# mnesbit/ImageExperiments

Hardware: AMD Instinct MI355X
Metric: encode Mpixels/s at quality=3.5 (higher is better)
Workload: dtype f64; 1 GPU; 4928x3264 synthetic RGB, 8 distinct frames in turn (mt19937 seed 12345+f), quality 3.5, K=32 atoms/tile-channel, 8x8 tiles; container_bytes=6650795

## Files before the change

### imageexperiments_amd/csrc/mp_pursuit.hip

```cpp
#include <hip/hip_runtime.h>
#include <stdint.h>
#include <type_traits>

#include "mp_device.h"

namespace mpc {

namespace {

constexpr int N = 64;
constexpr int kGroups = 1;
constexpr int kWavesDouble = 12;
constexpr int kWavesFloat = 12;
constexpr int kWavesMax = 16;
constexpr int kTilesLds = kBaseFilterTiles + kBlockFilterTiles;
constexpr double W_R = 0.299, W_G = 0.587, W_B = 0.114;
constexpr double U_SCALE = 0.436 / (1.0 - 0.114);
constexpr double V_SCALE = 0.615 / (1.0 - 0.299);
#ifndef MPC_SLACK
#define MPC_SLACK 0x1p-13f
#endif
constexpr float kSlack = MPC_SLACK;
constexpr float kAbs = 0x1p-100f;
constexpr float kHuge = 1.0e30f;
#ifndef MPC_REFILL_AT
#define MPC_REFILL_AT 16
#endif
constexpr int kRefillAt = MPC_REFILL_AT;

typedef float f32x4 __attribute__((ext_vector_type(4)));
typedef short bf16x8 __attribute__((ext_vector_type(8)));

template <int COUNT, class F>
__device__ __forceinline__ void static_for(F&& f)
{
    if constexpr (COUNT > 0) {
        static_for<COUNT - 1>(f);
        f(std::integral_constant<int, COUNT - 1>{});
    }
}

__device__ __forceinline__ unsigned short bf16_of(float x)
{
    const __bf16 b = static_cast<__bf16>(x);
    return __builtin_bit_cast(unsigned short, b);
}

template <class Op>
__device__ __forceinline__ unsigned reduce4_u(unsigned x, Op op)
{
    const auto a = __builtin_amdgcn_permlane16_swap(x, x, false, false);
    const unsigned m = op(a[0], a[1]);
    const auto b = __builtin_amdgcn_permlane32_swap(m, m, false, false);
    return op(b[0], b[1]);
}
__device__ __forceinline__ float reduce4_max(float x)
{
    return __uint_as_float(reduce4_u(__float_as_uint(x), [](unsigned p, unsigned q) {
        return __float_as_uint(__builtin_amdgcn_fmed3f(__uint_as_float(p), __uint_as_float(q), __builtin_inff()));
    }));
}
__device__ __forceinline__ unsigned reduce4_add(unsigned x) { return reduce4_u(x, [](unsigned p, unsigned q) { return p + q; }); }
__device__ __forceinline__ double reduce4_add(double x)
{
    unsigned lo = (unsigned)__double2loint(x), hi = (unsigned)__double2hiint(x);
    const auto a = __builtin_amdgcn_permlane16_swap(lo, lo, false, false);
    const auto b = __builtin_amdgcn_permlane16_swap(hi, hi, false, false);
    const double m = __hiloint2double((int)b[0], (int)a[0]) + __hiloint2double((int)b[1], (int)a[1]);
    lo = (unsigned)__double2loint(m); hi = (unsigned)__double2hiint(m);
    const auto c = __builtin_amdgcn_permlane32_swap(lo, lo, false, false);
    const auto d = __builtin_amdgcn_permlane32_swap(hi, hi, false, false);
    return __hiloint2double((int)d[0], (int)c[0]) + __hiloint2double((int)d[1], (int)c[1]);
}
__device__ __forceinline__ double from_prev16(double x)
{
    const unsigned lo = (unsigned)__double2loint(x), hi = (unsigned)__double2hiint(x);
    const auto a = __builtin_amdgcn_permlane16_swap(lo, lo, false, false);
    const auto b = __builtin_amdgcn_permlane16_swap(hi, hi, false, false);
    return __hiloint2double((int)b[0], (int)a[0]);
}
__device__ __forceinline__ double from_next16(double x)
{
    const unsigned lo = (unsigned)__double2loint(x), hi = (unsigned)__double2hiint(x);
    const auto a = __builtin_amdgcn_permlane16_swap(lo, lo, false, false);
    const auto b = __builtin_amdgcn_permlane16_swap(hi, hi, false, false);
    return __hiloint2double((int)b[1], (int)a[1]);
}
__device__ __forceinline__ double from_prev32(double x)
{
    const unsigned lo = (unsigned)__double2loint(x), hi = (unsigned)__double2hiint(x);
    const auto a = __builtin_amdgcn_permlane32_swap(lo, lo, false, false);
    const auto b = __builtin_amdgcn_permlane32_swap(hi, hi, false, false);
    return __hiloint2double((int)b[0], (int)a[0]);
}
__device__ __forceinline__ double from_next32(double x)
{
    const unsigned lo = (unsigned)__double2loint(x), hi = (unsigned)__double2hiint(x);
    const auto a = __builtin_amdgcn_permlane32_swap(lo, lo, false, false);
    const auto b = __builtin_amdgcn_permlane32_swap(hi, hi, false, false);
    return __hiloint2double((int)b[1], (int)a[1]);
}

__device__ __forceinline__ float from_prev16(float x) { return __uint_as_float(__builtin_amdgcn_permlane16_swap(__float_as_uint(x), __float_as_uint(x), false, false)[0]); }
__device__ __forceinline__ float from_next16(float x) { return __uint_as_float(__builtin_amdgcn_permlane16_swap(__float_as_uint(x), __float_as_uint(x), false, false)[1]); }
__device__ __forceinline__ float from_prev32(float x) { return __uint_as_float(__builtin_amdgcn_permlane32_swap(__float_as_uint(x), __float_as_uint(x), false, false)[0]); }
__device__ __forceinline__ float from_next32(float x) { return __uint_as_float(__builtin_amdgcn_permlane32_swap(__float_as_uint(x), __float_as_uint(x), false, false)[1]); }

__device__ __forceinline__ int pos_of(int h) { return h ^ (h >> 1); }

template <class T>
__device__ __forceinline__ T chain_sum(const T (&term)[16], int h)
{
    T t = 0;
#pragma unroll
    for (int i = 0; i < 16; ++i) t += term[i];
    T u = from_prev16(t);
#pragma unroll
    for (int i = 0; i < 16; ++i) u += term[i];
    t = h == 1 ? u : t;
    u = from_prev32(t);
#pragma unroll
    for (int i = 0; i < 16; ++i) u += term[i];
    t = h == 3 ? u : t;
    u = from_next16(t);
#pragma unroll
    for (int i = 0; i < 16; ++i) u += term[i];
    t = h == 2 ? u : t;
    u = from_prev16(t);
    t = h == 3 ? u : t;
    u = from_next32(t);
    return h < 2 ? u : t;
}

struct TopKeys {
    float k1 = 0.0f, k2 = 0.0f;
    __device__ __forceinline__ void see(unsigned value_bits, unsigned keep_mask, unsigned code)
    {
        const unsigned key = (value_bits & keep_mask) | code;
        k2 = __builtin_amdgcn_fmed3f(k1, k2, __uint_as_float(key));
        const unsigned k1b = __float_as_uint(k1);
        k1 = __uint_as_float(k1b > key ? k1b : key);
    }
};
__device__ __forceinline__ unsigned in_vgpr(unsigned x)
{
    unsigned v;
    asm volatile("v_mov_b32 %0, %1" : "=v"(v) : "s"(x));
    return v;
}
__device__ __forceinline__ unsigned in_sgpr(unsigned x)
{
    unsigned v;
    asm volatile("s_mov_b32 %0, %1" : "=s"(v) : "s"(x));
    return v;
}
constexpr unsigned kKeepRow = 0x7FFFFF80u;
constexpr unsigned kKeepPair = 0x7FFFFE00u;

struct Survivors {
    int q0 = 0, q1 = 0, q2 = 0, q3 = 0, count = 0;
    bool overflow = false;
    __device__ __forceinline__ void push(int code)
    {
        if (count == 0) q0 = code; else if (count == 1) q1 = code; else if (count == 2) q2 = code; else if (count == 3) q3 = code;
        else overflow = true;
        if (count < 4) ++count;
    }
    __device__ __forceinline__ int at(int i) const { return i == 0 ? q0 : (i == 1 ? q1 : (i == 2 ? q2 : q3)); }
};

struct TileChannel {
    int prev_id = 0;
    int next_off = 0;
    int off0 = 0;
    int npairs = 0;
    int fresh = -1;
    unsigned pk0 = 0, pk1 = 0;
    unsigned swept = 0;
    bool has0 = false, live = false;
    double coeff = 0.0;
    int sel_g = 0;
    int step = 0;
    int t = 0;
    __device__ __forceinline__ unsigned packed(int p) const { return ((p < 2 ? pk0 : pk1) >> (16 * (p & 1))) & 0xFFFFu; }
};

__device__ __forceinline__ void load16(double (&x)[16], const double* p)
{
    const double2* q = reinterpret_cast<const double2*>(p);
#pragma unroll
    for (int i = 0; i < 8; ++i) {
        const double2 v = q[i];
        x[2 * i] = v.x;
        x[2 * i + 1] = v.y;
// ... 18 lines not shown

template <class T>
__device__ __forceinline__ void keep_better(T& v, int& i, int& sel, T ov, int oi, int osel)
{
    const T a = abs_of(ov), b = abs_of(v);
    if (oi >= 0 && (a > b || (a == b && i >= 0 && oi < i))) {
        v = ov; i = oi; sel = osel;
    }
}

__device__ __forceinline__ int lane_id_fresh()
{
    int l;
    asm volatile("v_mbcnt_lo_u32_b32 %0, -1, 0\n\tv_mbcnt_hi_u32_b32 %0, -1, %0" : "=v"(l));
    return l;
}
#define FRESH_LANE                                                                    \
    const int lane = lane_id_fresh();                                                 \
    const int slot = lane & 15, h = lane >> 4;                                        \
    const int pix0 = 16 * pos_of(h);                                                  \
    (void)slot; (void)h; (void)pix0;

#ifdef MPC_STAMPS
#define STAMP(i)                                              \
    {                                                         \
        __builtin_amdgcn_sched_barrier(0);                    \
        const unsigned long long now_ = __builtin_amdgcn_s_memtime(); \
        __builtin_amdgcn_sched_barrier(0);                    \
        stamp_acc[i] += now_ - stamp_prev;                    \
        stamp_prev = now_;                                    \
    }
#define COUNT(i, n) stamp_acc[i] += (unsigned long long)(n);
#else
#define STAMP(i)
#define COUNT(i, n)
#endif

}

template <class T, int kWaves>
__global__ __launch_bounds__(64 * kWaves, kWaves / 4) void mp_pursuit_kernel(const PursuitArgs a)
{
    constexpr bool kFast = std::is_same<T, float>::value;
#ifdef MPC_STAMPS
    unsigned long long stamp_acc[24];
    for (int i = 0; i < 24; ++i) stamp_acc[i] = 0;
    unsigned long long stamp_prev = __builtin_amdgcn_s_memtime();
    const unsigned long long wg_begin = __builtin_amdgcn_s_memrealtime();
#endif
    __shared__ uint4 s_tiles[kTilesLds * 256];
    __shared__ int s_rows[512], s_rowoff[512];
    __shared__ unsigned s_touch[64 * kWaves];
    __shared__ double s_quant[3][kMaxDeviceK];
    __shared__ int s_home;
    __shared__ int s_on[3];
    const int ch_first = a.n_tc[0] > 0 ? 0 : (a.n_tc[1] > 0 ? 1 : 2);
    const T* const base_rows = reinterpret_cast<const T*>(kFast ? static_cast<const void*>(a.base32) : static_cast<const void*>(a.base));
    {
        const uint16_t* const blk0 = ch_first == 0 ? a.block_tiles[0] : (ch_first == 1 ? a.block_tiles[1] : a.block_tiles[2]);
        const uint4* src_base = reinterpret_cast<const uint4*>(a.base_tiles);
        const uint4* src_blk0 = reinterpret_cast<const uint4*>(blk0);
        for (int i = threadIdx.x; i < kTilesLds * 256; i += 64 * kWaves)
            s_tiles[i] = i < kBaseFilterTiles * 256 ? src_base[i] : src_blk0[i - kBaseFilterTiles * 256];
        for (int i = threadIdx.x; i < 512; i += 64 * kWaves) {
            s_rows[i] = i < a.num_base ? a.block_rows[i] : 0;
            s_rowoff[i] = i < a.num_base ? a.block_row_off[i] : 0;
        }
        for (int i = threadIdx.x; i < 3 * kMaxDeviceK; i += 64 * kWaves)
            s_quant[i / kMaxDeviceK][i % kMaxDeviceK] = (i % kMaxDeviceK) < a.K ? a.quant[(i / kMaxDeviceK) * a.K + i % kMaxDeviceK] : 1.0;
        if (threadIdx.x == 0) {
            s_home = ch_first;
            s_on[0] = s_on[1] = s_on[2] = 0;
            s_on[ch_first] = kWaves;
        }
    }
    __syncthreads();

    const int wave = __builtin_amdgcn_readfirstlane((int)(threadIdx.x >> 6));
    int ch = ch_first;
    const T* detail = nullptr;
    const uint16_t* block_tiles = nullptr;
    const float* gram = nullptr;
    unsigned* queue = nullptr;
    long long n_tc = 0;
    auto bind_channel = [&](int c) {
        c = __builtin_amdgcn_readfirstlane(c);
        ch = c;
        detail = reinterpret_cast<const T*>(kFast ? static_cast<const void*>(c == 0 ? a.detail32[0] : (c == 1 ? a.detail32[1] : a.detail32[2]))
                                                  : static_cast<const void*>(c == 0 ? a.detail[0] : (c == 1 ? a.detail[1] : a.detail[2])));
        block_tiles = c == 0 ? a.block_tiles[0] : (c == 1 ? a.block_tiles[1] : a.block_tiles[2]);
        gram = c == 0 ? a.gram[0] : (c == 1 ? a.gram[1] : a.gram[2]);
        queue = a.queue + c;
        n_tc = c == 0 ? a.n_tc[0] : (c == 1 ? a.n_tc[1] : a.n_tc[2]);
    };
    bind_channel(ch_first);
    const long long wave_global = (long long)blockIdx.x * kWaves + wave;
    float* const my_p = a.pair_p + wave_global * (kGroups * 16 * kMaxPairs * 64);
    unsigned* const my_meta = a.pair_meta + wave_global * (kGroups * 16 * kMaxPairs * 2);
    float* const my_e = a.pair_e + wave_global * (kGroups * 16 * kMaxPairs);
    unsigned* const my_touch = s_touch + 64 * wave;
    const int K = a.K;

    const unsigned keep_row_mask = in_vgpr(kKeepRow), keep_pair_mask = in_vgpr(kKeepPair);
    unsigned n_mfma = 0, n_steps = 0;
    int unit[kGroups];
    T r[kGroups][16];
    TileChannel tc[kGroups];
#pragma unroll
    for (int g = 0; g < kGroups; ++g) {
        unit[g] = -1;
#pragma unroll
        for (int i = 0; i < 16; ++i) r[g][i] = 0;
    }
    bool queue_empty = false;

    auto tile_mfma = [&](const uint4 (&av)[4], const bf16x8 (&hi)[2], const bf16x8 (&lo)[2]) {
        f32x4 acc = {0.0f, 0.0f, 0.0f, 0.0f};
#pragma unroll
        for (int kk = 0; kk < 2; ++kk) {
            bf16x8 ah, al;
            __builtin_memcpy(&ah, &av[2 * kk + 0], 16);
            __builtin_memcpy(&al, &av[2 * kk + 1], 16);
            acc = __builtin_amdgcn_mfma_f32_16x16x32_bf16(ah, hi[kk], acc, 0, 0, 0);
            acc = __builtin_amdgcn_mfma_f32_16x16x32_bf16(ah, lo[kk], acc, 0, 0, 0);
            acc = __builtin_amdgcn_mfma_f32_16x16x32_bf16(al, hi[kk], acc, 0, 0, 0);
        }
        return acc;
    };
    auto rec_of = [&](int t) { return a.vec_in ? (long long)t : (long long)t * 3 + ch; };
    auto lds_tile = [&](uint4 (&dst)[4], int t, int lane) {
#pragma unroll
        for (int q = 0; q < 4; ++q) dst[q] = s_tiles[t * 256 + q * 64 + lane];
    };
    auto far_tile = [&](uint4 (&dst)[4], int t, int lane) {
        const uint4* tiles = reinterpret_cast<const uint4*>(block_tiles) + lane;
#pragma unroll
        for (int q = 0; q < 4; ++q) dst[q] = tiles[t * 256 + q * 64];
    };

    TopKeys tp[kGroups];
    float lbmax[kGroups];
    bool oddp[kGroups];
    float rbound[kGroups];
#pragma unroll
    for (int g = 0; g < kGroups; ++g) { lbmax[g] = -3.0e38f; oddp[g] = false; rbound[g] = 0.0f; }
    auto pair_update = [&](auto gc, auto same_p, int p, bool upd, unsigned info, float4 (&pv)[4], const float4 (&gv)[4], float E) {
        constexpr int g = decltype(gc)::value;
        FRESH_LANE
        const long long pi = (long long)(g * 16 + slot) * kMaxPairs + p;
        const int rows = (int)((info >> 9) & 127u);
        if (upd) {
            const float c32 = (float)tc[g].coeff;
            float4* pp = reinterpret_cast<float4*>(my_p + pi * 64 + 4 * h);
#pragma unroll
            for (int t = 0; t < 4; ++t) {
                pv[t].x = fmaf(-c32, gv[t].x, pv[t].x);
                pv[t].y = fmaf(-c32, gv[t].y, pv[t].y);
                pv[t].z = fmaf(-c32, gv[t].z, pv[t].z);
                pv[t].w = fmaf(-c32, gv[t].w, pv[t].w);
                pp[4 * t] = pv[t];
            }
            E = (E + 0x1p-21f * (fabsf(c32) + rbound[g])) * 1.000001f;
            if (h == 0) my_e[pi] = E;
            oddp[g] = oddp[g] || !(fabsf(c32) < kHuge);
        }
        oddp[g] = oddp[g] || !(E < kHuge);
        const bool pad2 = h == 3 && rows < 63, pad3 = h == 3 && rows < 64;
        const unsigned keepp = keep_pair_mask;
        float biggest = 0.0f;
#pragma unroll
        for (int t = 0; t < 4; ++t) {
            const float vals[4] = {pv[t].x, pv[t].y, pv[t].z, pv[t].w};
#pragma unroll
            for (int v = 0; v < 4; ++v) {
                const float m = fabsf(vals[v]);
                float ub = m + E;
                if (t == 3 && v == 2) ub = pad2 ? 0.0f : ub;
                if (t == 3 && v == 3) ub = pad3 ? 0.0f : ub;
                const unsigned code = (unsigned)((p << 4) | (t << 2) | v);
                tp[g].see(__float_as_uint(ub), keepp, decltype(same_p)::value ? in_sgpr((unsigned)__builtin_amdgcn_readfirstlane((int)code)) : code);
                biggest = __builtin_amdgcn_fmed3f(biggest, m, __builtin_inff());
            }
        }
        lbmax[g] = __builtin_amdgcn_fmed3f(lbmax[g], biggest - E, __builtin_inff());
    };
    for (;;) {
        bool any_unit = false;
        for (;;) {
        static_for<kGroups>([&](auto gc) {
            constexpr int g = decltype(gc)::value;
            if (queue_empty) return;
            const unsigned free_slots = (unsigned)(__ballot(!tc[g].live) & 0xFFFFull);
            const int n_free = __popc(free_slots);
            if (!(n_free >= kRefillAt || (unit[g] < 0 && n_free > 0))) return;
            FRESH_LANE
            int first = 0;
            if (lane == 0) first = (int)atomicAdd(queue, (unsigned)n_free);
            first = __builtin_amdgcn_readfirstlane(first);
            if ((long long)first + n_free >= n_tc) queue_empty = true;
            const long long t = (long long)first + __popc(free_slots & ((1u << slot) - 1u));
            const bool take = !tc[g].live && t < n_tc;
            if (!__ballot(take)) return;
            unit[g] = 0;
            TileChannel s;
            s.live = true;
            s.t = (int)t;
            s.next_off = a.num_base;
            const long long ts = take ? t : 0;
            T fresh_r[16];
            if (a.vec_in) {
                double in[16];
                load16(in, a.vec_in + ts * N + pix0);
#pragma unroll
                for (int i = 0; i < 16; ++i) fresh_r[i] = (T)in[i];
            } else {
                const int tiles_per_frame = a.tiles_x * a.tile_rows;
                const int frame = (int)(ts / tiles_per_frame);
                const int tile = (int)(ts - (long long)frame * tiles_per_frame);
                const int tx = tile / a.tile_rows, ty = a.tile_row_begin + (tile - tx * a.tile_rows);
                if (a.out_tile_rows > 0) s.t = (frame * a.tiles_x + tx) * a.out_tile_rows + ty;
                const uint8_t* img = a.rgb + (long long)frame * a.frame_stride;
                unsigned char px[16][3];
                const bool whole = tx * 8 + 8 <= a.width && ty * 8 + 8 <= a.height;
                if (a.rgb_aligned8 && !__ballot(!whole)) {
#pragma unroll
                    for (int rr = 0; rr < 2; ++rr) {
                        const uint2* p = reinterpret_cast<const uint2*>(img + (long long)(ty * 8 + (pix0 >> 3) + rr) * a.row_stride + 24 * tx);
                        const uint2 v0 = p[0], v1 = p[1], v2 = p[2];
                        const unsigned w[6] = {v0.x, v0.y, v1.x, v1.y, v2.x, v2.y};
#pragma unroll
                        for (int b = 0; b < 24; ++b) px[8 * rr + b / 3][b % 3] = (unsigned char)((w[b >> 2] >> (8 * (b & 3))) & 0xFFu);
                    }
                } else {
// ... 73 lines not shown
            ss = reduce4_add(ss);
            nz[g] = reduce4_add(nzl ? 1u : 0u) != 0u;
            rnorm[g] = (float)__builtin_sqrt(ss) * 1.0000002f;
            Eb[g] = kSlack * rnorm[g] + kAbs;
            rbound[g] = rnorm[g];
            odd[g] = !(rnorm[g] < kHuge);
        });
        STAMP(1)

        static_for<kGroups>([&](auto gc) {
            constexpr int g = decltype(gc)::value;
            if (unit[g] < 0) return;
            const bool mine = tc[g].live && tc[g].fresh >= 0;
            unsigned long long pend = __ballot(mine) & 0xFFFFull;
            if (!pend) return;
            FRESH_LANE
            COUNT(19, __popcll(pend))
            unsigned fresh_info = 0;
            if (mine)
                fresh_info = (tc[g].fresh < 4 ? tc[g].packed(tc[g].fresh) : my_meta[2 * ((long long)(g * 16 + slot) * kMaxPairs + tc[g].fresh)]) & 0xFFFFu;
            float4 pnew[4];
#pragma unroll
            for (int t = 0; t < 4; ++t) pnew[t] = make_float4(0.0f, 0.0f, 0.0f, 0.0f);
            while (pend) {
                const int src = __builtin_ctzll(pend);
                pend &= pend - 1;
                const int blk = __builtin_amdgcn_readlane((int)(fresh_info & 511u), src);
                n_mfma += 6 * kBlockFilterTiles;
                const uint4* tiles = reinterpret_cast<const uint4*>(block_tiles) + (long long)blk * (kBlockFilterTiles * 256) + lane;
#ifndef MPC_NEWPAIR_TILES
#define MPC_NEWPAIR_TILES 2
#endif
                constexpr int kInFlight = MPC_NEWPAIR_TILES;
#pragma unroll
                for (int t2 = 0; t2 < kBlockFilterTiles; t2 += kInFlight) {
                    uint4 av[kInFlight][4];
#pragma unroll
                    for (int t = 0; t < kInFlight; ++t)
#pragma unroll
                        for (int q = 0; q < 4; ++q) av[t][q] = tiles[(t2 + t) * 256 + q * 64];
#pragma unroll
                    for (int t = 0; t < kInFlight; ++t) {
                        const f32x4 acc = tile_mfma(av[t], bh[g], bl[g]);
                        if (slot == src) pnew[t2 + t] = make_float4(acc[0], acc[1], acc[2], acc[3]);
                    }
                }
            }
            if (mine) {
                float4* dst = reinterpret_cast<float4*>(my_p + ((long long)(g * 16 + slot) * kMaxPairs + tc[g].fresh) * 64 + 4 * h);
#pragma unroll
                for (int t = 0; t < 4; ++t) dst[4 * t] = pnew[t];
                if (h == 0) my_e[(g * 16 + slot) * kMaxPairs + tc[g].fresh] = Eb[g];
                const float4 none[4] = {};
                pair_update(gc, std::false_type{}, tc[g].fresh, false, fresh_info, pnew, none, Eb[g]);
            }
        });
        STAMP(3)

        TopKeys tb[kGroups], td[kGroups];
        bool any0 = false;
#pragma unroll
        for (int g = 0; g < kGroups; ++g) any0 = any0 || (unit[g] >= 0 && __ballot(tc[g].live && tc[g].has0) != 0);
        n_mfma += 6 * kGroups * (kBaseFilterTiles + (any0 ? kBlockFilterTiles : 0));
        {
            FRESH_LANE
            uint4 ta[4];
            f32x4 acc[kGroups], prev[kGroups];
            const unsigned keep = keep_row_mask;
            auto track = [&](TopKeys (&trk)[kGroups], const f32x4 (&val)[kGroups], unsigned code0) {
                unsigned code[4];
#pragma unroll
                for (int v = 0; v < 4; ++v) code[v] = (unsigned)__builtin_amdgcn_readfirstlane((int)(code0 + v));
#pragma unroll
                for (int g = 0; g < kGroups; ++g)
#pragma unroll
                    for (int v = 0; v < 4; ++v) trk[g].see(__float_as_uint(val[g][v]), keep, code[v]);
            };
            lds_tile(ta, 0, lane);
#pragma unroll
            for (int g = 0; g < kGroups; ++g) prev[g] = tile_mfma(ta, bh[g], bl[g]);
#pragma unroll 1
            for (int t = 1; t < kBaseFilterTiles - 1; t += 2) {
                lds_tile(ta, t, lane);
#pragma unroll
                for (int g = 0; g < kGroups; ++g) acc[g] = tile_mfma(ta, bh[g], bl[g]);
                track(tb, prev, 4 * (t - 1));
                lds_tile(ta, t + 1, lane);
#pragma unroll
                for (int g = 0; g < kGroups; ++g) prev[g] = tile_mfma(ta, bh[g], bl[g]);
                track(tb, acc, 4 * t);
            }
            lds_tile(ta, kBaseFilterTiles - 1, lane);
#pragma unroll
            for (int g = 0; g < kGroups; ++g) acc[g] = tile_mfma(ta, bh[g], bl[g]);
            track(tb, prev, 4 * (kBaseFilterTiles - 2));
            track(tb, acc, 4 * (kBaseFilterTiles - 1));
            if (any0) {
#pragma unroll 1
                for (int t = 0; t < kBlockFilterTiles; ++t) {
                    if (home) lds_tile(ta, kBaseFilterTiles + t, lane);
                    else far_tile(ta, t, lane);
#pragma unroll
                    for (int g = 0; g < kGroups; ++g) acc[g] = tile_mfma(ta, bh[g], bl[g]);
                    track(td, acc, 4 * t);
                }
            }
        }
        STAMP(4)

        Survivors sv[kGroups];
        float thr_b[kGroups], Tmin[kGroups];
        bool pass2[kGroups], rescan[kGroups];
        static_for<kGroups>([&](auto gc) {
            constexpr int g = decltype(gc)::value;
            pass2[g] = false; rescan[g] = false; thr_b[g] = 0.0f; Tmin[g] = 0.0f;
            if (unit[g] < 0) return;
            FRESH_LANE
            const bool has0 = tc[g].has0, hasp = tc[g].npairs > 0;
            const float top_b = __uint_as_float(__float_as_uint(reduce4_max(tb[g].k1)) & kKeepRow);
            const float top_d = __uint_as_float(__float_as_uint(reduce4_max(td[g].k1)) & kKeepRow);
            const float lbm = reduce4_max(lbmax[g]);
            const bool bad = odd[g] || (hasp && reduce4_add(oddp[g] ? 1u : 0u) != 0u);
            float t = top_b - Eb[g];
            if (has0) t = fmaxf(t, top_d - Eb[g]);
            if (hasp) t = fmaxf(t, lbm);
            Tmin[g] = bad ? -__builtin_inff() : t;
            thr_b[g] = (Tmin[g] - Eb[g]) * (1.0f - 0x1p-15f);
            const float thr_p = Tmin[g] * (1.0f - 0x1p-13f);
            const bool live = tc[g].live && nz[g];
            const bool vague = bad || !(thr_b[g] > 0.0f);
            const bool unclear_b = vague || !(tb[g].k2 < thr_b[g]) || (has0 && !(td[g].k2 < thr_b[g]));
            const bool unclear_p = hasp && (vague || !(tp[g].k2 < thr_p));
            pass2[g] = __ballot(live && unclear_b) != 0;
            rescan[g] = live && reduce4_add(unclear_p ? 1u : 0u) != 0u;
            if (live && !pass2[g]) {
                if (!(tb[g].k1 < thr_b[g])) {
                    const unsigned code = __float_as_uint(tb[g].k1) & 127u;
                    sv[g].push((int)(16 * (code >> 2) + 4 * h + (code & 3u)));
                }
                if (has0 && !(td[g].k1 < thr_b[g])) {
                    const unsigned code = __float_as_uint(td[g].k1) & 127u;
                    sv[g].push((1 << 16) | (int)(16 * (code >> 2) + 4 * h + (code & 3u)));
                }
            }
            if (live && hasp && !rescan[g] && !(tp[g].k1 < thr_p)) {
                const unsigned code = __float_as_uint(tp[g].k1) & 511u;
                sv[g].push((2 << 16) | (int)((code >> 4) << 11) | (int)(16 * ((code >> 2) & 3u) + 4 * h + (code & 3u)));
            }
        });
        STAMP(5)

        bool any2 = false;
#pragma unroll
        for (int g = 0; g < kGroups; ++g) any2 = any2 || pass2[g];
        if (any2) {
            static_for<kGroups>([&](auto gc) { COUNT(13, pass2[decltype(gc)::value] ? 1 : 0) });
            FRESH_LANE
            uint4 cur[4], nxt[4];
            lds_tile(cur, 0, lane);
            const int last = any0 ? kTilesLds : kBaseFilterTiles;
            auto any_tile = [&](uint4 (&dst)[4], int t) {
                if (t < kBaseFilterTiles || home) lds_tile(dst, t, lane);
                else far_tile(dst, t - kBaseFilterTiles, lane);
            };
            static_for<kGroups>([&](auto gc) { n_mfma += pass2[decltype(gc)::value] ? 6 * last : 0; });
#pragma unroll 1
            for (int t = 0; t < last; ++t) {
                any_tile(nxt, t + 1 < last ? t + 1 : t);
                const bool is_base = t < kBaseFilterTiles;
                const int row0 = (is_base ? t : t - kBaseFilterTiles) * 16 + 4 * h;
                const int limit = is_base ? a.num_base : a.rows0;
                static_for<kGroups>([&](auto gc) {
                    constexpr int g = decltype(gc)::value;
                    if (!pass2[g]) return;
                    const f32x4 acc = tile_mfma(cur, bh[g], bl[g]);
                    const bool wanted = tc[g].live && nz[g] && (is_base || tc[g].has0);
#pragma unroll
                    for (int v = 0; v < 4; ++v)
                        if (wanted && !(fabsf(acc[v]) < thr_b[g]) && row0 + v < limit) sv[g].push((is_base ? 0 : (1 << 16)) | (row0 + v));
                });
#pragma unroll
                for (int q = 0; q < 4; ++q) cur[q] = nxt[q];
            }
        }
        STAMP(6)
        static_for<kGroups>([&](auto gc) {
            constexpr int g = decltype(gc)::value;
            if (unit[g] < 0 || !__ballot(rescan[g])) return;
            FRESH_LANE
            for (int p = 0; __ballot(rescan[g] && p < tc[g].npairs) != 0; ++p) {
                if (!(rescan[g] && p < tc[g].npairs)) continue;
                const long long pi = (long long)(g * 16 + slot) * kMaxPairs + p;
                const int rows = (int)((my_meta[2 * pi] >> 9) & 127u);
                const float E = my_e[pi];
                const float4* pp = reinterpret_cast<const float4*>(my_p + pi * 64 + 4 * h);
#pragma unroll
                for (int t = 0; t < 4; ++t) {
                    const float4 x = pp[4 * t];
                    const float vals[4] = {x.x, x.y, x.z, x.w};
#pragma unroll
                    for (int v = 0; v < 4; ++v) {
                        const int row = 16 * t + 4 * h + v;
                        if (row < rows && !(fabsf(vals[v]) + E < Tmin[g])) sv[g].push((2 << 16) | (p << 11) | row);
                    }
                }
            }
        });
        STAMP(7)

        T best_val[kGroups];
        int best_idx[kGroups], best_sel[kGroups];
        int c0[kGroups], c1[kGroups], c2[kGroups], total[kGroups];
        bool exhaustive[kGroups];
        const int lane7 = lane_id_fresh();
        const int slot7 = lane7 & 15, h7 = lane7 >> 4, pix7 = 16 * pos_of(h7);
#pragma unroll
        for (int g = 0; g < kGroups; ++g) {
            best_val[g] = 0; best_idx[g] = -1; best_sel[g] = 0;
            c0[g] = __shfl(sv[g].count, slot7);
            c1[g] = __shfl(sv[g].count, slot7 + 16);
            c2[g] = __shfl(sv[g].count, slot7 + 32);
            total[g] = c0[g] + c1[g] + c2[g] + __shfl(sv[g].count, slot7 + 48);
            exhaustive[g] = reduce4_add(sv[g].overflow ? 1u : 0u) != 0u;
        }
        auto resolve = [&](auto gc, int code, const T*& ptr, int& idx, int& sel) {
            constexpr int g = decltype(gc)::value;
            const int seg = code >> 16, row = code & 2047;
            if (seg == 0) { ptr = base_rows + (long long)row * N; idx = row; sel = row; }
            else if (seg == 1) { ptr = detail + (long long)row * N; idx = tc[g].off0 + row; sel = a.num_base + row; }
            else {
                const int p = (code >> 11) & 31;
                const long long pi = (long long)(g * 16 + slot7) * kMaxPairs + p;
                const unsigned meta = my_meta[2 * pi];
                const int drow = s_rowoff[meta & 511u] + row;
                ptr = detail + (long long)drow * N;
                idx = (int)(meta >> 16) + row;
                sel = a.num_base + drow;
            }
        };
        auto evaluate2 = [&](const bool (&on)[kGroups], const int (&code)[kGroups]) {
            const T* ptr[kGroups];
            int idx[kGroups], sel[kGroups];
            T x[kGroups][16];
            static_for<kGroups>([&](auto gc) {
                constexpr int g = decltype(gc)::value;
                ptr[g] = base_rows; idx[g] = -1; sel[g] = 0;
                if (on[g]) resolve(gc, code[g], ptr[g], idx[g], sel[g]);
            });
#pragma unroll
            for (int g = 0; g < kGroups; ++g) load16(x[g], ptr[g] + pix7);
#pragma unroll
            for (int g = 0; g < kGroups; ++g)
#pragma unroll
                for (int i = 0; i < 16; ++i) x[g][i] = x[g][i] * r[g][i];
            T p[kGroups];
#pragma unroll
            for (int g = 0; g < kGroups; ++g) p[g] = chain_sum(x[g], h7);
#pragma unroll
            for (int g = 0; g < kGroups; ++g)
                if (on[g]) keep_better(best_val[g], best_idx[g], best_sel[g], p[g], idx[g], sel[g]);
        };
        for (int k = 0;; ++k) {
            bool on[kGroups];
            int code[kGroups];
            bool any = false;
#pragma unroll
            for (int g = 0; g < kGroups; ++g) {
                on[g] = unit[g] >= 0 && tc[g].live && !exhaustive[g] && k < total[g];
                any = any || on[g];
                const int owner = k < c0[g] ? 0 : (k < c0[g] + c1[g] ? 1 : (k < c0[g] + c1[g] + c2[g] ? 2 : 3));
                const int local = k - (owner == 0 ? 0 : (owner == 1 ? c0[g] : (owner == 2 ? c0[g] + c1[g] : c0[g] + c1[g] + c2[g])));
                code[g] = __shfl(sv[g].at(local & 3), slot7 + 16 * owner);
            }
            if (!__ballot(any)) break;
            COUNT(14, 1)
            evaluate2(on, code);
        }
// ... 14 lines not shown
                    bool on[kGroups];
                    int code[kGroups];
                    bool more = false, any = false;
                    static_for<kGroups>([&](auto gc) {
                        constexpr int g = decltype(gc)::value;
                        on[g] = ex[g] && n < n_all[g];
                        more = more || on[g];
                        code[g] = 0;
                        if (n < a.num_base) code[g] = n;
                        else if (n < a.num_base + 64) { code[g] = (1 << 16) | (n - a.num_base); on[g] = on[g] && tc[g].has0 && n - a.num_base < a.rows0; }
                        else {
                            const int p = (n - a.num_base - 64) >> 6, row = (n - a.num_base - 64) & 63;
                            code[g] = (2 << 16) | (p << 11) | row;
                            if (on[g]) on[g] = row < (int)((my_meta[2 * ((long long)(g * 16 + slot7) * kMaxPairs + p)] >> 9) & 127u);
                        }
                        any = any || on[g];
                    });
                    if (!__ballot(more)) break;
                    if (!__ballot(any)) continue;
                    evaluate2(on, code);
                }
            }
        }
        STAMP(9)

        T xrow[kGroups][16];
#pragma unroll
        for (int g = 0; g < kGroups; ++g) {
            FRESH_LANE
            const int sg = (unit[g] >= 0 && tc[g].live && best_idx[g] >= 0) ? best_sel[g] : 0;
            load16(xrow[g], (sg < a.num_base ? base_rows + (long long)sg * N : detail + (long long)(sg - a.num_base) * N) + pix0);
        }
        bool ended[kGroups];
        static_for<kGroups>([&](auto gc) {
            constexpr int g = decltype(gc)::value;
            ended[g] = false;
            if (unit[g] < 0) return;
            FRESH_LANE
            TileChannel& s = tc[g];
            s.coeff = 0.0;
            s.fresh = -1;
            if (!s.live) return;
            s.swept += (unsigned)s.next_off;
            int count = 0;
            unsigned record = 0;
            if (best_idx[g] < 0) {
                ended[g] = true; count = s.step;
            } else {
                const int id = best_idx[g];
                const unsigned delta = s.step > 0 ? (((unsigned)(id - s.prev_id) << 1) ^ (unsigned)((id - s.prev_id) >> 31)) : (unsigned)id;
                s.prev_id = id;
                const T qstep = (T)s_quant[ch][s.step];
                const T ratio = best_val[g] / qstep;
                const int q = kFast ? (int)__builtin_roundf((float)ratio) : (int)__builtin_round((double)ratio);
                const unsigned zz = ((unsigned)q << 1) ^ (unsigned)(q >> 31);
                record = (delta & 0xFFFFu) | ((zz & 0xFFFFu) << 16);
                if (q == 0) {
                    ended[g] = true; count = s.step;
                } else {
                    s.coeff = (double)(qstep * (T)q);
                    s.sel_g = best_sel[g];
                    if (s.step + 1 == K) { ended[g] = true; count = K; }
                    else if (id < a.num_base) {
                        const int rows = s_rows[id];
                        bool repeat = id == 0 && s.has0;
                        for (int p = 0; p < s.npairs; ++p) {
                            const unsigned blk = p < 4 ? (s.packed(p) & 511u) : (my_meta[2 * ((long long)(g * 16 + slot) * kMaxPairs + p)] & 511u);
                            repeat = repeat || (int)blk == id;
                        }
                        if (!repeat) {
                            if (id == 0) { s.has0 = true; s.off0 = s.next_off; }
                            else {
                                const long long pi = (long long)(g * 16 + slot) * kMaxPairs + s.npairs;
                                const unsigned info = (unsigned)id | ((unsigned)rows << 9);
                                if (h == 0) my_meta[2 * pi] = info | ((unsigned)s.next_off << 16);
                                if (s.npairs < 2) s.pk0 |= info << (16 * s.npairs);
                                else if (s.npairs < 4) s.pk1 |= info << (16 * (s.npairs - 2));
                                s.fresh = s.npairs;
                                s.npairs += 1;
                            }
                        }
                        s.next_off += rows;
                    }
                }
            }
            if (h == 0) {
                const long long rec = rec_of(s.t);
                a.out.choices[rec * K + s.step] = record;
                if (ended[g]) {
                    a.out.counts[rec] = (uint16_t)count;
                    if (a.out.swept) a.out.swept[rec] = s.swept;
                }
            }
        });
        STAMP(10)

        float4 pv0[kGroups][4], gv0[kGroups][4];
        float E0[kGroups];
        bool on0[kGroups], upd0[kGroups];
        unsigned info0[kGroups];
#pragma unroll
        for (int g = 0; g < kGroups; ++g) {
            FRESH_LANE
            on0[g] = unit[g] >= 0 && tc[g].live && !ended[g] && tc[g].npairs > 0 && tc[g].fresh != 0;
            upd0[g] = on0[g] && tc[g].coeff != 0.0;
            info0[g] = tc[g].packed(0);
            const long long pi = (long long)(g * 16 + slot) * kMaxPairs;
            const float4* pp = reinterpret_cast<const float4*>(my_p + pi * 64 + 4 * h);
            const float4* gp = reinterpret_cast<const float4*>(gram + (upd0[g] ? (long long)tc[g].sel_g * a.gram_stride + (int)(info0[g] & 511u) * 64 : 0) + 4 * h);
#pragma unroll
            for (int t = 0; t < 4; ++t) { pv0[g][t] = pp[4 * t]; gv0[g][t] = gp[4 * t]; }
            E0[g] = my_e[pi];
        }
#pragma unroll
        for (int g = 0; g < kGroups; ++g) { tp[g] = TopKeys(); lbmax[g] = -3.0e38f; oddp[g] = false; }
        static_for<kGroups>([&](auto gc) {
            constexpr int g = decltype(gc)::value;
            if (__ballot(on0[g])) { COUNT(17, 1) COUNT(18, __popcll(__ballot(on0[g]) & 0xFFFFull)) }
            if (on0[g]) pair_update(gc, std::true_type{}, 0, upd0[g], info0[g], pv0[g], gv0[g], E0[g]);
        });
#pragma unroll 1
        for (int p = 1;; ++p) {
            bool on[kGroups];
            bool any = false;
#pragma unroll
            for (int g = 0; g < kGroups; ++g) {
                on[g] = unit[g] >= 0 && tc[g].live && !ended[g] && p < tc[g].npairs && p != tc[g].fresh;
                any = any || (unit[g] >= 0 && tc[g].live && !ended[g] && p < tc[g].npairs);
            }
            if (!__ballot(any)) break;
            unsigned info[kGroups];
            float4 pv[kGroups][4], gv[kGroups][4];
            float E[kGroups];
            bool upd[kGroups];
#pragma unroll
            for (int g = 0; g < kGroups; ++g) {
                FRESH_LANE
                const long long pi = (long long)(g * 16 + slot) * kMaxPairs + (on[g] ? p : 0);
                info[g] = p < 4 ? tc[g].packed(p) : (my_meta[2 * pi] & 0xFFFFu);
                upd[g] = on[g] && tc[g].coeff != 0.0;
                const float4* pp = reinterpret_cast<const float4*>(my_p + pi * 64 + 4 * h);
                const float4* gp = reinterpret_cast<const float4*>(gram + (upd[g] ? (long long)tc[g].sel_g * a.gram_stride + (int)(info[g] & 511u) * 64 : 0) + 4 * h);
#pragma unroll
                for (int t = 0; t < 4; ++t) { pv[g][t] = pp[4 * t]; gv[g][t] = gp[4 * t]; }
                E[g] = my_e[pi];
            }
            static_for<kGroups>([&](auto gc) {
                constexpr int g = decltype(gc)::value;
                COUNT(17, 1) COUNT(18, __popcll(__ballot(on[g]) & 0xFFFFull))
                if (on[g]) pair_update(gc, std::true_type{}, p, upd[g], info[g], pv[g], gv[g], E[g]);
            });
        }
        STAMP(2)


        static_for<kGroups>([&](auto gc) {
            constexpr int g = decltype(gc)::value;
            if (unit[g] < 0) return;
            FRESH_LANE
            TileChannel& s = tc[g];
            const bool upd = s.live && s.coeff != 0.0;
            if (upd) {
#pragma unroll
                for (int i = 0; i < 16; ++i) {
                    const T scaled = (T)s.coeff * xrow[g][i];
                    r[g][i] = r[g][i] - scaled;
                }
            }
            if (a.out.energy && __ballot(s.live && ended[g])) {
                T sq[16];
#pragma unroll
                for (int i = 0; i < 16; ++i) sq[i] = r[g][i] * r[g][i];
                const T e2 = chain_sum(sq, h);
                if (s.live && ended[g] && h == 0) a.out.energy[rec_of(s.t)] = (double)e2;
            }
            unsigned long long pend = __ballot(s.live && !ended[g] && s.fresh >= 0 && s.fresh < 4 && h == 0);
            while (pend) {
                const int src = __builtin_ctzll(pend);
                pend &= pend - 1;
                const int blk = __builtin_amdgcn_readlane((int)(s.packed(s.fresh >= 0 && s.fresh < 4 ? s.fresh : 0) & 511u), src);
                const uint16_t* tiles = block_tiles + (long long)blk * (kBlockFilterTiles * 2048) + 64 * lane;
                __builtin_amdgcn_global_load_lds(tiles, my_touch, 4, 0, 0);
                __builtin_amdgcn_global_load_lds(tiles + 4096, my_touch, 4, 0, 0);
            }
            if (ended[g]) s.live = false;
            s.step += 1;
            if (!__ballot(s.live)) unit[g] = -1;
        });
        STAMP(11)
    }
    FRESH_LANE
    if (lane == 0 && a.stats) {
        atomicAdd(a.stats + 0, (unsigned long long)n_mfma);
        atomicAdd(a.stats + 1, (unsigned long long)n_steps);
    }
#ifdef MPC_STAMPS
    if (lane == 0 && a.debug)
        for (int i = 0; i < 24; ++i) atomicAdd(a.debug + i, stamp_acc[i]);
    if (lane == 0 && a.debug && blockIdx.x < 1024) {
        atomicMin(a.debug + 24 + 2 * blockIdx.x, wg_begin);
        atomicMax(a.debug + 25 + 2 * blockIdx.x, (unsigned long long)__builtin_amdgcn_s_memrealtime());
    }
#endif
}
// ... 71 lines not shown
```

### imageexperiments_amd/csrc/mpcodec_context.cpp

```cpp
#include <algorithm>
#include <chrono>
#include <cmath>
#include <cstdarg>
#include <cstdio>
#include <cstring>

#include "mpc_internal.h"

namespace {
thread_local char g_error[512] = "";

template <class T>
hipError_t upload(T** dst, const T* src, size_t count) {
    hipError_t e = hipMalloc(reinterpret_cast<void**>(dst), count * sizeof(T));
    if (e != hipSuccess) return e;
    return hipMemcpy(*dst, src, count * sizeof(T), hipMemcpyHostToDevice);
}
}

mpc_status fail(mpc_status st, const char* fmt, ...) {
    va_list ap;
    va_start(ap, fmt);
    vsnprintf(g_error, sizeof g_error, fmt, ap);
    va_end(ap);
// ... 212 lines not shown
        p.mem = nullptr;
        hipError_t e = hipMalloc(&p.mem, bytes);
        if (e != hipSuccess) { c->ws_cap = 0; return fail(MPC_ERR_ALLOC, "workspace of %zu bytes: %s", bytes, hipGetErrorString(e)); }
        p.ws = mpc::carve_workspace(p.mem, static_cast<int>(cap), c->K);
    }
    c->ws_cap = static_cast<int>(cap);
    return MPC_OK;
}

constexpr int kBaseParts = 8;
constexpr int kRowParts = 4;

namespace {
hipError_t timing_events(mpc_context* c, size_t n, hipEvent_t** ev) {
    if (!c->timing) return hipSuccess;
    const size_t need = c->timing_used + n;
    while (c->timing_events.size() < need) {
        hipEvent_t e;
        if (const hipError_t err = hipEventCreate(&e); err != hipSuccess) return err;
        c->timing_events.push_back(e);
    }
    *ev = c->timing_events.data() + c->timing_used;
    c->timing_used = need;
    return hipSuccess;
}

#ifdef MPC_STAMPS
constexpr int kDebugWords = 24 + 2 * 1024;

hipError_t stamps_reset(hipStream_t s, unsigned long long** debug) {
    static unsigned long long* d_debug = nullptr;
    hipError_t e = d_debug ? hipSuccess : hipMalloc(reinterpret_cast<void**>(&d_debug), kDebugWords * sizeof(unsigned long long));
    std::vector<unsigned long long> init(kDebugWords, 0ULL);
    for (int b = 0; b < 1024; ++b) init[24 + 2 * b] = ~0ULL;
    if (e == hipSuccess) e = hipStreamSynchronize(s);
    if (e == hipSuccess) e = hipMemcpy(d_debug, init.data(), kDebugWords * sizeof(unsigned long long), hipMemcpyHostToDevice);
    *debug = d_debug;
    return e;
}

hipError_t stamps_report(hipStream_t s, const unsigned long long* d_debug, int workgroups, int cus) {
    std::vector<unsigned long long> all(kDebugWords);
    hipError_t e = hipStreamSynchronize(s);
    if (e == hipSuccess) e = hipMemcpy(all.data(), d_debug, kDebugWords * sizeof(unsigned long long), hipMemcpyDeviceToHost);
    if (e != hipSuccess) return e;
    const unsigned long long* hst = all.data();
    unsigned long long tot = 0;
    for (int i = 0; i < 12; ++i) tot += hst[i];
    std::fprintf(stderr, "[stamps wg%d] wave-steps %llu live-lanes/step %.1f pass2-groups %llu rounds %llu exhaustive %llu | cycles/wave-step:",
                 workgroups, hst[12], hst[12] ? (double)hst[16] / hst[12] / 4.0 : 0.0, hst[13], hst[14], hst[15]);
    for (int i = 0; i < 12; ++i) std::fprintf(stderr, " %d:%.0f", i, hst[12] ? (double)hst[i] / hst[12] : 0.0);
    std::fprintf(stderr, " total %.0f | pair rounds/step %.2f slots/round %.2f new pairs/step %.2f\n", hst[12] ? (double)tot / hst[12] : 0.0,
                 hst[12] ? (double)hst[17] / hst[12] : 0.0, hst[17] ? (double)hst[18] / hst[17] : 0.0, hst[12] ? (double)hst[19] / hst[12] : 0.0);
    const int grid = workgroups;
    unsigned long long t0 = ~0ULL, t1 = 0;
    for (int b = 0; b < grid && b < 1024; ++b) { t0 = std::min(t0, all[24 + 2 * b]); t1 = std::max(t1, all[25 + 2 * b]); }
    if (t1 > t0) {
        const double span = (double)(t1 - t0);
        double busy = 0.0;
        int slices[20] = {};
        for (int b = 0; b < grid && b < 1024; ++b) {
            busy += (double)(all[25 + 2 * b] - all[24 + 2 * b]);
            for (int k = 0; k < 20; ++k) {
                const double mid = t0 + span * (k + 0.5) / 20.0;
                if ((double)all[24 + 2 * b] <= mid && mid < (double)all[25 + 2 * b]) ++slices[k];
            }
        }
        std::fprintf(stderr, "[residency] span %.1f us, workgroup-time / (%d CUs x span) = %.3f | resident workgroups per 5 %% slice:", span / 100.0,
                     cus, busy / (span * cus));
        for (int k = 0; k < 20; ++k) std::fprintf(stderr, " %d", slices[k]);
        std::fprintf(stderr, "\n");
    }
    return hipSuccess;
}
#endif

mpc_status run_persistent(mpc_context* c, const Tuning& t, const mpc::FrameInput& in, const mpc::Outputs& out, const double* d_quant,
                          long long total_tc, void* stream) {
    DeviceDict& d = *c->dd;
    hipStream_t s = static_cast<hipStream_t>(stream);
    const bool vec = in.vec_in != nullptr;
    const long long n_tc = vec ? total_tc : total_tc / 3;
    const long long n_units = (n_tc + 15) / 16 * (vec ? 1 : 3);
    if (n_tc >= (1LL << 31)) return fail(MPC_ERR_ARGUMENT, "batch too large");
    const int per_wg = mpc::pursuit_units_per_workgroup();
    int workgroups = static_cast<int>(std::min<long long>((n_units + per_wg - 1) / per_wg, d.workgroups));
    if (const int limit = c->seq_workgroups.load(std::memory_order_relaxed); limit > 0) workgroups = std::min(workgroups, limit);
    if (const int limit = c->user_workgroups.load(std::memory_order_relaxed); limit > 0) workgroups = std::min(workgroups, limit);
    if (t.workgroups > 0) workgroups = std::min(t.workgroups, d.workgroups);
    std::lock_guard<std::mutex> hold(d.launch_lock);
    HIP_TRY(hipStreamWaitEvent(s, d.done[0], 0));
    HIP_TRY(hipMemsetAsync(d.queues, 0, 3 * sizeof(unsigned), s));
    const long long n_sel = d.num_base + d.detail_rows, stride = static_cast<long long>(d.num_base) * 64;
    mpc::PursuitArgs a{};
    a.base = d.d_base;
    a.base32 = d.d_base32;

    a.fast = c->fast ? 1 : 0;
    a.base_tiles = d.d_base_t1;
    for (int ch = 0; ch < 3; ++ch) {
        a.detail[ch] = d.d_detail + static_cast<size_t>(ch) * d.detail_rows * mpc::kTileN;
        a.detail32[ch] = d.d_detail32 + static_cast<size_t>(ch) * d.detail_rows * mpc::kTileN;
        a.block_tiles[ch] = d.d_detail_t1 + static_cast<size_t>(ch) * d.num_base * mpc::kBlockFilterTiles * mpc::kFilterTileHalves;
        a.gram[ch] = d.d_gram + static_cast<size_t>(ch) * n_sel * stride;
        a.n_tc[ch] = vec ? (ch == in.vec_channel ? n_tc : 0) : n_tc;
    }
// ... 456 lines not shown
```

Measured before the change: 5303 Mpixels/s.

## Decide quantized coefficient from float bounds when only one candidate survives

When a tile-channel has exactly one surviving candidate, this computes a bounded float estimate of its correlation (bf16-split dot product from LDS tiles, or the tracked pair energy for pair rows). If both interval ends quantize to the same integer, the coefficient is taken as decided and the exact double-precision resolve round is skipped. To support this it keeps per-lane pair energies and the first few pair metadata entries in LDS, which adds LDS use, register pressure and extra stores on every step. Correctness depends on the interval bounds being conservative.

```diff
diff --git a/imageexperiments_amd/csrc/mp_pursuit.hip b/imageexperiments_amd/csrc/mp_pursuit.hip
--- a/imageexperiments_amd/csrc/mp_pursuit.hip
+++ b/imageexperiments_amd/csrc/mp_pursuit.hip
@@ -27,6 +27,12 @@
 #define MPC_REFILL_AT 16
 #endif
 constexpr int kRefillAt = MPC_REFILL_AT;
+#ifdef MPC_ALWAYS_EXACT
+constexpr bool kDecide = false;
+#else
+constexpr bool kDecide = true;
+#endif
+constexpr int kLdsPairs = 4;
 
 typedef float f32x4 __attribute__((ext_vector_type(4)));
 typedef short bf16x8 __attribute__((ext_vector_type(8)));
@@ -61,6 +67,10 @@
     }));
 }
 __device__ __forceinline__ unsigned reduce4_add(unsigned x) { return reduce4_u(x, [](unsigned p, unsigned q) { return p + q; }); }
+__device__ __forceinline__ float reduce4_add(float x)
+{
+    return __uint_as_float(reduce4_u(__float_as_uint(x), [](unsigned p, unsigned q) { return __float_as_uint(__uint_as_float(p) + __uint_as_float(q)); }));
+}
 __device__ __forceinline__ double reduce4_add(double x)
 {
     unsigned lo = (unsigned)__double2loint(x), hi = (unsigned)__double2hiint(x);
@@ -140,6 +150,18 @@
         k2 = __builtin_amdgcn_fmed3f(k1, k2, __uint_as_float(key));
         const unsigned k1b = __float_as_uint(k1);
         k1 = __uint_as_float(k1b > key ? k1b : key);
+    }
+};
+struct TopPairKeys : TopKeys {
+    float e1 = 0.0f;
+    __device__ __forceinline__ void see(unsigned value_bits, unsigned keep_mask, unsigned code, float p, float e)
+    {
+        const unsigned key = (value_bits & keep_mask) | code;
+        k2 = __builtin_amdgcn_fmed3f(k1, k2, __uint_as_float(key));
+        const unsigned k1b = __float_as_uint(k1);
+        const bool top = key > k1b;
+        k1 = __uint_as_float(top ? key : k1b);
+        e1 = top ? __builtin_copysignf(e, p) : e1;
     }
 };
 __device__ __forceinline__ unsigned in_vgpr(unsigned x)
@@ -264,6 +286,8 @@
     __shared__ int s_rows[512], s_rowoff[512];
     __shared__ unsigned s_touch[64 * kWaves];
     __shared__ double s_quant[3][kMaxDeviceK];
+    __shared__ unsigned s_pmeta[kWaves * kGroups * 16 * kLdsPairs];
+    __shared__ float s_e1[kWaves * kGroups * 64];
     __shared__ int s_home;
     __shared__ int s_on[3];
     const int ch_first = a.n_tc[0] > 0 ? 0 : (a.n_tc[1] > 0 ? 1 : 2);
@@ -311,6 +335,8 @@
     unsigned* const my_meta = a.pair_meta + wave_global * (kGroups * 16 * kMaxPairs * 2);
     float* const my_e = a.pair_e + wave_global * (kGroups * 16 * kMaxPairs);
     unsigned* const my_touch = s_touch + 64 * wave;
+    unsigned* const my_pmeta = s_pmeta + kGroups * 16 * kLdsPairs * wave;
+    float* const my_e1 = s_e1 + kGroups * 64 * wave;
     const int K = a.K;
 
     const unsigned keep_row_mask = in_vgpr(kKeepRow), keep_pair_mask = in_vgpr(kKeepPair);
@@ -350,7 +376,7 @@
         for (int q = 0; q < 4; ++q) dst[q] = tiles[t * 256 + q * 64];
     };
 
-    TopKeys tp[kGroups];
+    TopPairKeys tp[kGroups];
     float lbmax[kGroups];
     bool oddp[kGroups];
     float rbound[kGroups];
@@ -390,7 +416,8 @@
                 if (t == 3 && v == 2) ub = pad2 ? 0.0f : ub;
                 if (t == 3 && v == 3) ub = pad3 ? 0.0f : ub;
                 const unsigned code = (unsigned)((p << 4) | (t << 2) | v);
-                tp[g].see(__float_as_uint(ub), keepp, decltype(same_p)::value ? in_sgpr((unsigned)__builtin_amdgcn_readfirstlane((int)code)) : code);
+                tp[g].see(__float_as_uint(ub), keepp, decltype(same_p)::value ? in_sgpr((unsigned)__builtin_amdgcn_readfirstlane((int)code)) : code,
+                          vals[v], E);
                 biggest = __builtin_amdgcn_fmed3f(biggest, m, __builtin_inff());
             }
         }
@@ -570,7 +597,9 @@
                 for (int t = 0; t < 4; ++t) dst[4 * t] = pnew[t];
                 if (h == 0) my_e[(g * 16 + slot) * kMaxPairs + tc[g].fresh] = Eb[g];
                 const float4 none[4] = {};
+                if (kDecide) tp[g].e1 = my_e1[g * 64 + lane];
                 pair_update(gc, std::false_type{}, tc[g].fresh, false, fresh_info, pnew, none, Eb[g]);
+                if (kDecide) my_e1[g * 64 + lane] = tp[g].e1;
             }
         });
         STAMP(3)
@@ -628,10 +657,10 @@
 
         Survivors sv[kGroups];
         float thr_b[kGroups], Tmin[kGroups];
-        bool pass2[kGroups], rescan[kGroups];
+        bool pass2[kGroups], rescan[kGroups], bad_g[kGroups];
         static_for<kGroups>([&](auto gc) {
             constexpr int g = decltype(gc)::value;
-            pass2[g] = false; rescan[g] = false; thr_b[g] = 0.0f; Tmin[g] = 0.0f;
+            pass2[g] = false; rescan[g] = false; bad_g[g] = true; thr_b[g] = 0.0f; Tmin[g] = 0.0f;
             if (unit[g] < 0) return;
             FRESH_LANE
             const bool has0 = tc[g].has0, hasp = tc[g].npairs > 0;
@@ -639,6 +668,7 @@
             const float top_d = __uint_as_float(__float_as_uint(reduce4_max(td[g].k1)) & kKeepRow);
             const float lbm = reduce4_max(lbmax[g]);
             const bool bad = odd[g] || (hasp && reduce4_add(oddp[g] ? 1u : 0u) != 0u);
+            bad_g[g] = bad;
             float t = top_b - Eb[g];
             if (has0) t = fmaxf(t, top_d - Eb[g]);
             if (hasp) t = fmaxf(t, lbm);
@@ -741,6 +771,86 @@
             total[g] = c0[g] + c1[g] + c2[g] + __shfl(sv[g].count, slot7 + 48);
             exhaustive[g] = reduce4_add(sv[g].overflow ? 1u : 0u) != 0u;
         }
+        bool decided[kGroups];
+        int dq[kGroups];
+        static_for<kGroups>([&](auto gc) {
+            constexpr int g = decltype(gc)::value;
+            decided[g] = false; dq[g] = 0;
+            if (!kDecide || unit[g] < 0) return;
+            const bool one = tc[g].live && nz[g] && !bad_g[g] && !exhaustive[g] && total[g] == 1;
+            if (!__ballot(one)) return;
+            const int code = (int)reduce4_add(sv[g].count > 0 ? (unsigned)sv[g].q0 : 0u);
+            const int seg = code >> 16, row = code & 2047, pair = (code >> 11) & 31;
+            const bool mfma_row = seg == 0 || (seg == 1 && home);
+            float part = 0.0f;
+            if (one && mfma_row) {
+                const int tile = (seg == 0 ? 0 : kBaseFilterTiles) + (row >> 4);
+                uint4 tv[4];
+#pragma unroll
+                for (int q = 0; q < 4; ++q) tv[q] = s_tiles[tile * 256 + q * 64 + (row & 15) + 16 * h7];
+                float acc2[2] = {0.0f, 0.0f};
+#pragma unroll
+                for (int kk = 0; kk < 2; ++kk) {
+                    const unsigned wh[4] = {tv[2 * kk].x, tv[2 * kk].y, tv[2 * kk].z, tv[2 * kk].w};
+                    const unsigned wl[4] = {tv[2 * kk + 1].x, tv[2 * kk + 1].y, tv[2 * kk + 1].z, tv[2 * kk + 1].w};
+#pragma unroll
+                    for (int j = 0; j < 8; ++j) {
+                        const float ah = __uint_as_float((j & 1) ? (wh[j >> 1] & 0xFFFF0000u) : (wh[j >> 1] << 16));
+                        const float al = __uint_as_float((j & 1) ? (wl[j >> 1] & 0xFFFF0000u) : (wl[j >> 1] << 16));
+                        T rj = r[g][8 * kk + j];
+                        asm volatile("" : "+v"(rj));
+                        const float x = (float)rj;
+                        const float rh = __uint_as_float((unsigned)bf16_of(x) << 16);
+                        const float rl = __uint_as_float((unsigned)bf16_of(x - rh) << 16);
+                        acc2[kk] = fmaf(ah, rh, acc2[kk]);
+                        acc2[kk] = fmaf(ah, rl, acc2[kk]);
+                        acc2[kk] = fmaf(al, rh, acc2[kk]);
+                    }
+                }
+                part = acc2[0] + acc2[1];
+            }
+            const bool mine = sv[g].count > 0;
+            const float cb = reduce4_add(part);
+            const float kt = reduce4_add(mine ? __uint_as_float(__float_as_uint(tp[g].k1) & kKeepPair) : 0.0f);
+            const float es = reduce4_add(mine ? my_e1[g * 64 + lane7] : 0.0f);
+            const bool pair_row = seg == 2 && !rescan[g] && pair < kLdsPairs;
+            const float Eb_g = kSlack * rbound[g] + kAbs;
+            const bool neg = mfma_row ? cb < 0.0f : es < 0.0f;
+            const double ca = (double)fabsf(cb), eb = (double)Eb_g, kd = (double)kt, ep = (double)fabsf(es);
+            const double lo = (mfma_row ? ca - eb : kd * (1.0 - 0x1p-24) - 2.0 * ep) * (1.0 - 0x1p-50);
+            const double hi = (mfma_row ? ca + eb : kd * (1.0 + 0x1p-13)) * (1.0 + 0x1p-50);
+            T lo_t, hi_t;
+            if constexpr (kFast) { lo_t = __double2float_rd(lo); hi_t = __double2float_ru(hi); }
+            else { lo_t = lo; hi_t = hi; }
+            const T qstep = (T)s_quant[ch][tc[g].step];
+            T rl, rh;
+            if constexpr (kFast) { rl = __builtin_roundf(lo_t / qstep); rh = __builtin_roundf(hi_t / qstep); }
+            else { rl = __builtin_round(lo_t / qstep); rh = __builtin_round(hi_t / qstep); }
+            decided[g] = one && (mfma_row || pair_row) && lo_t > (T)0 && rl == rh;
+            if (!decided[g]) return;
+            dq[g] = (int)(neg ? -rl : rl);
+            total[g] = 0;
+            if (seg == 0) { best_idx[g] = row; best_sel[g] = row; }
+            else if (seg == 1) { best_idx[g] = tc[g].off0 + row; best_sel[g] = a.num_base + row; }
+            else {
+                const unsigned meta = my_pmeta[(g * 16 + slot7) * kLdsPairs + pair];
+                best_idx[g] = (int)(meta >> 16) + row;
+                best_sel[g] = a.num_base + s_rowoff[meta & 511u] + row;
+            }
+        });
+#ifdef MPC_STAMPS
+        {
+            int all_rounds = 0;
+            for (int k = 0; k < 16; ++k) {
+                bool need = false;
+#pragma unroll
+                for (int g = 0; g < kGroups; ++g) need = need || (unit[g] >= 0 && tc[g].live && !exhaustive[g] && k < (decided[g] ? 1 : total[g]));
+                all_rounds += __ballot(need) != 0 ? 1 : 0;
+            }
+            COUNT(21, all_rounds)
+            static_for<kGroups>([&](auto gc) { COUNT(20, __popcll(__ballot(decided[decltype(gc)::value]) & 0xFFFFull)) });
+        }
+#endif
         auto resolve = [&](auto gc, int code, const T*& ptr, int& idx, int& sel) {
             constexpr int g = decltype(gc)::value;
             const int seg = code >> 16, row = code & 2047;
@@ -861,7 +971,7 @@
                 s.prev_id = id;
                 const T qstep = (T)s_quant[ch][s.step];
                 const T ratio = best_val[g] / qstep;
-                const int q = kFast ? (int)__builtin_roundf((float)ratio) : (int)__builtin_round((double)ratio);
+                const int q = decided[g] ? dq[g] : (kFast ? (int)__builtin_roundf((float)ratio) : (int)__builtin_round((double)ratio));
                 const unsigned zz = ((unsigned)q << 1) ^ (unsigned)(q >> 31);
                 record = (delta & 0xFFFFu) | ((zz & 0xFFFFu) << 16);
                 if (q == 0) {
@@ -883,6 +993,7 @@
                                 const long long pi = (long long)(g * 16 + slot) * kMaxPairs + s.npairs;
                                 const unsigned info = (unsigned)id | ((unsigned)rows << 9);
                                 if (h == 0) my_meta[2 * pi] = info | ((unsigned)s.next_off << 16);
+                                if (kDecide && h == 0 && s.npairs < kLdsPairs) my_pmeta[(g * 16 + slot) * kLdsPairs + s.npairs] = info | ((unsigned)s.next_off << 16);
                                 if (s.npairs < 2) s.pk0 |= info << (16 * s.npairs);
                                 else if (s.npairs < 4) s.pk1 |= info << (16 * (s.npairs - 2));
                                 s.fresh = s.npairs;
@@ -922,7 +1033,7 @@
             E0[g] = my_e[pi];
         }
 #pragma unroll
-        for (int g = 0; g < kGroups; ++g) { tp[g] = TopKeys(); lbmax[g] = -3.0e38f; oddp[g] = false; }
+        for (int g = 0; g < kGroups; ++g) { tp[g] = TopPairKeys(); lbmax[g] = -3.0e38f; oddp[g] = false; }
         static_for<kGroups>([&](auto gc) {
             constexpr int g = decltype(gc)::value;
             if (__ballot(on0[g])) { COUNT(17, 1) COUNT(18, __popcll(__ballot(on0[g]) & 0xFFFFull)) }
@@ -959,6 +1070,11 @@
                 COUNT(17, 1) COUNT(18, __popcll(__ballot(on[g]) & 0xFFFFull))
                 if (on[g]) pair_update(gc, std::true_type{}, p, upd[g], info[g], pv[g], gv[g], E[g]);
             });
+        }
+        if (kDecide) {
+            FRESH_LANE
+#pragma unroll
+            for (int g = 0; g < kGroups; ++g) my_e1[g * 64 + lane] = tp[g].e1;
         }
         STAMP(2)
 
diff --git a/imageexperiments_amd/csrc/mpcodec_context.cpp b/imageexperiments_amd/csrc/mpcodec_context.cpp
--- a/imageexperiments_amd/csrc/mpcodec_context.cpp
+++ b/imageexperiments_amd/csrc/mpcodec_context.cpp
@@ -288,6 +288,8 @@
     for (int i = 0; i < 12; ++i) std::fprintf(stderr, " %d:%.0f", i, hst[12] ? (double)hst[i] / hst[12] : 0.0);
     std::fprintf(stderr, " total %.0f | pair rounds/step %.2f slots/round %.2f new pairs/step %.2f\n", hst[12] ? (double)tot / hst[12] : 0.0,
                  hst[12] ? (double)hst[17] / hst[12] : 0.0, hst[17] ? (double)hst[18] / hst[17] : 0.0, hst[12] ? (double)hst[19] / hst[12] : 0.0);
+    std::fprintf(stderr, "[stamps wg%d] exact rounds/step %.3f (without deciding %.3f) decided slots/step %.2f\n", workgroups,
+                 hst[12] ? (double)hst[14] / hst[12] : 0.0, hst[12] ? (double)hst[21] / hst[12] : 0.0, hst[12] ? (double)hst[20] / hst[12] : 0.0);
     const int grid = workgroups;
     unsigned long long t0 = ~0ULL, t1 = 0;
     for (int b = 0; b < grid && b < 1024; ++b) { t0 = std::min(t0, all[24 + 2 * b]); t1 = std::max(t1, all[25 + 2 * b]); }
```

Result: no change. 5342 Mpixels/s, median of 6 (+0.7%).
